# CPJKU/audio_sheet_retrieval

Measured on AMD Instinct MI355X. Metric: snippet-pairs/sec embedded+ranked (32-d CCA), higher is better.
Workload: dtype f32

## Files before the change

### audio_sheet_retrieval_amd/csrc/asr_api.hip

```cpp
#include "asr_ctx.h"


namespace asr_detail {

thread_local std::string g_create_error;

int fail(asr_ctx *ctx, int code, const char *fmt, ...) {
    char buf[512];
    va_list ap;
    va_start(ap, fmt);
    vsnprintf(buf, sizeof buf, fmt, ap);
    va_end(ap);
    if (ctx) ctx->err = buf; else g_create_error = buf;
    return code;
}


void build_geometry(Tower &t, int nf, int H, int W) {
    const int ch[9][2] = {{1, nf}, {nf, nf}, {nf, 2 * nf}, {2 * nf, 2 * nf}, {2 * nf, 4 * nf},
                          {4 * nf, 4 * nf}, {4 * nf, 4 * nf}, {4 * nf, 4 * nf}, {4 * nf, 32}};
    t.in_h = H; t.in_w = W;
    int h = H, w = W;
    for (int b = 0; b < 9; ++b) {
        LayerGeom &g = t.g[b];
// ... 98 lines not shown
    if (T.mask) hipFree(T.mask);
    if (T.raw1) hipFree(T.raw1);
    if (T.repack_dev) hipFree(T.repack_dev);
    if (T.cca_ws) hipFree(T.cca_ws);
    if (T.l2_dev) hipFree(T.l2_dev);
    if (T.cca_done) hipEventDestroy(T.cca_done);
    for (hipEvent_t e : T.gate) if (e) hipEventDestroy(e);
    ctx->train.reset();
}

void free_comm(asr_ctx *ctx) {
    if (!ctx->comm) return;
    Comm &c = *ctx->comm;
    for (auto &pr : c.timed) { (void)hipEventDestroy(pr.first); (void)hipEventDestroy(pr.second); }
    c.timed.clear();
    if (c.nccl && c.pCommDestroy) (void)c.pCommDestroy(c.nccl);
    if (c.dl) dlclose(c.dl);
    ctx->comm.reset();
    ctx->exch = asr::Exchange{};
}

void free_pipe(asr_ctx *ctx) {
    auto &P = ctx->pipe;
    for (int s = 0; s < 2; ++s) {
        void *bufs[] = {P.in1[s], P.in2[s], P.lv1[s], P.lv2[s], P.ranks[s], P.ties[s], P.dstar[s]};
        for (void *b : bufs) if (b) (void)hipFree(b);
        hipEvent_t evs[] = {P.ready[s], P.done[s], P.out[s]};
        for (hipEvent_t e : evs) if (e) (void)hipEventDestroy(e);
    }
    if (P.h2d && P.h2d != ctx->copy_streams[0]) (void)hipStreamDestroy(P.h2d);
    if (P.d2h && P.d2h != ctx->copy_streams[1]) (void)hipStreamDestroy(P.d2h);
    P = asr_ctx::Pipe{};
}

void free_hpipe(asr_ctx *ctx) {
    auto &H = ctx->hpipe;
    for (int s = 0; s < asr_ctx::HostPipe::NSLOT; ++s) {
        if (H.pin[s]) (void)hipHostFree(H.pin[s]);
        if (H.dev[s]) (void)hipFree(H.dev[s]);
        if (H.copied[s]) (void)hipEventDestroy(H.copied[s]);
        if (H.consumed[s]) (void)hipEventDestroy(H.consumed[s]);
        H.pin[s] = H.dev[s] = nullptr; H.copied[s] = H.consumed[s] = nullptr; H.used[s] = false;
    }
    H.slot_bytes = 0;
    if (H.out_dev) (void)hipFree(H.out_dev);
    H.out_dev = nullptr; H.out_floats = 0;
    if (H.h2d && H.h2d != ctx->copy_streams[2]) (void)hipStreamDestroy(H.h2d);
    H.h2d = nullptr;
    H.pool.reset();
}

void free_ctx_buffers(asr_ctx *ctx) {
    free_train(ctx);
    free_comm(ctx);
    free_pipe(ctx);
    free_hpipe(ctx);
    for (auto &t : ctx->tw) {
        for (int b = 0; b < 9; ++b) { if (t.w_dev[b]) hipFree(t.w_dev[b]); if (t.bn_dev[b]) hipFree(t.bn_dev[b]); }
        for (int b = 0; b < 8; ++b) if (t.act[b]) hipFree(t.act[b]);
    }
    if (ctx->cca_dev) hipFree(ctx->cca_dev);
    for (int v = 0; v < 2; ++v) {
        if (ctx->in_stage[v]) hipFree(ctx->in_stage[v]);
        if (ctx->out_stage[v]) hipFree(ctx->out_stage[v]);
        if (ctx->vdone[v]) hipEventDestroy(ctx->vdone[v]);
        if (ctx->vstream[v]) hipStreamDestroy(ctx->vstream[v]);
    }
    if (ctx->main_done) hipEventDestroy(ctx->main_done);
    if (ctx->wside_stream) { (void)hipStreamSynchronize(ctx->wside_stream); (void)hipStreamDestroy(ctx->wside_stream); }
    for (hipStream_t &cs : ctx->copy_streams)
        if (cs) { (void)hipStreamSynchronize(cs); (void)hipStreamDestroy(cs); cs = nullptr; }
    if (ctx->norm1) hipFree(ctx->norm1);
    if (ctx->norm2) hipFree(ctx->norm2);
    if (ctx->cca_ws) hipFree(ctx->cca_ws);
    if (ctx->topk_ws) hipFree(ctx->topk_ws);
    if (ctx->topk_tickets) hipFree(ctx->topk_tickets);
    if (ctx->unit_ws) hipFree(ctx->unit_ws);
    if (ctx->rank_io) hipFree(ctx->rank_io);
    if (ctx->valid_ws) hipFree(ctx->valid_ws);
    for (auto &r : ctx->prof) prof_fold(r.get());
    if (ctx->stream) hipStreamDestroy(ctx->stream);
}

hipError_t launch_conv_any(asr_ctx *ctx, hipStream_t st, const asr::ConvPlan &p, const float *in, const float *w,
                           const float *bn, float *out, int n, const asr::Fuse1Args *f1, double *stats, int *stats_rows,
                           bool stats_clean, const asr::BnBwdFuse *bf) {
    if (stats_rows) *stats_rows = 0;
    if (p.variant >= 4000)
        return asr::launch_conv_wino4(st, p, in, w + asr::conv_wpack_floats(p.cin, p.cout) + asr::wino_wpack_floats(p.cin, p.cout),
                                      bn, out, n, ctx->num_cus, stats, stats_rows, stats_clean, bf);
    if (p.variant >= 3000)
        return asr::launch_conv_wino(st, p, in, w + asr::conv_wpack_floats(p.cin, p.cout), bn, out, n, ctx->num_cus,
                                     stats, stats_rows, p.fuse1 ? f1 : nullptr, stats_clean, bf);
    if (p.variant >= 2000) return asr::launch_conv_v3(st, p, in, w, bn, out, n, ctx->num_cus, p.fuse1 ? f1 : nullptr);
    return p.variant >= 1000 ? asr::launch_conv_v2(st, p, in, w, bn, out, n, ctx->num_cus)
                             : asr::launch_conv(st, p, in, w, bn, out, n, ctx->num_cus, f1);
}

int tune_cache_tag() {
    static int tag = -1;
    if (tag < 0) {
        unsigned h = 2166136261u;
        for (const char *p = asr_version(); *p; ++p) h = (h ^ (unsigned char)*p) * 16777619u;
        tag = (int)(h & 0x7fffffffu);
    }
    return tag;
}

int autotune_tower(asr_ctx *ctx, int view) {
    Tower &t = ctx->tw[view - 1];
    hipStream_t st = ctx->estream[view - 1];
    const int n = ctx->chunk;
    hipEvent_t e0, e1;
    ASR_HIP(ctx, hipEventCreate(&e0));
    ASR_HIP(ctx, hipEventCreate(&e1));
    const bool dbg = getenv("ASR_DEBUG") != nullptr;
    for (int b = 1; b < 8; ++b) {
        const LayerGeom &g = t.g[b];
        std::vector<asr::ConvPlan> cands;
        cands.push_back(t.plan[b]);
        const char *fenv = getenv("ASR_FUSE1");
        const bool forced = (b == 1 && t.fuse1);
        const bool try_fused = (b == 1) && fenv && fenv[0] != '0' && fenv[0] != 'w' && getenv("ASR_NO_FUSE1") == nullptr;
        const bool try_wfused = (b == 1) && !(fenv && fenv[0] == '0') && getenv("ASR_NO_FUSE1") == nullptr &&
                                !(view == 1 && ctx->cfg.resize_view1) && !forced;
        const bool only_wfused = try_wfused && fenv && fenv[0] == 'w';
        if (!forced) {
            asr::conv_candidates_v1(g.cin, g.cout, g.pool, g.H, g.W, 0, 5, &cands, 0);
            asr::conv_candidates_v2(g.cin, g.cout, g.pool, g.H, g.W, 5, &cands);
            asr::conv_candidates_v3(g.cin, g.cout, g.pool, g.H, g.W, 6, &cands, 0);
            asr::conv_candidates_wino(g.cin, g.cout, g.pool, g.H, g.W,
                                      getenv("ASR_WINO_CANDS") ? atoi(getenv("ASR_WINO_CANDS")) : 4, &cands);
            asr::conv_candidates_wino4(g.cin, g.cout, g.pool, g.H, g.W, &cands);
        } else {
            asr::conv_candidates_v1(g.cin, g.cout, g.pool, g.H, g.W, 0, 5, &cands, 1);
        }
        if (try_fused) asr::conv_candidates_v3(g.cin, g.cout, g.pool, g.H, g.W, 6, &cands, 1);
        if (try_wfused) {
            asr::conv_candidates_wino_fused(g.cin, g.cout, g.pool, g.H, g.W, 3, &cands);
            if (only_wfused) {
                std::vector<asr::ConvPlan> only;
                for (auto &c : cands)
                    if (c.variant >= 3000 && c.variant < 3500 && c.fuse1) only.push_back(c);
                if (!only.empty()) cands.swap(only);
            }
        }
        if (b == 1 && fenv && fenv[0] == '3') {
            std::vector<asr::ConvPlan> only;
            for (auto &c : cands)
                if (c.variant >= 2000 && c.fuse1) only.push_back(c);
            if (!only.empty()) cands.swap(only);
        }
        if (const char *only_env = getenv("ASR_TUNE_ONLY")) {
            const int lo = !strcmp(only_env, "wino4") ? 4000 : !strcmp(only_env, "winog") ? 3500 : !strcmp(only_env, "wino") ? 3000 : 0;
            const int hi = !strcmp(only_env, "wino4") ? 5000 : !strcmp(only_env, "winog") ? 4000 : !strcmp(only_env, "wino") ? 3500 : 3000;
            std::vector<asr::ConvPlan> only;
            for (auto &c : cands)
                if (c.variant >= lo && c.variant < hi) only.push_back(c);
            if (!only.empty()) cands.swap(only);
        }
        asr::Fuse1Args f1{t.act[0], t.w_dev[0], t.bn_dev[0], ASR_IN_F32_PREPARED, 0, g.H, g.W};
        const asr::Fuse1Args *pf1 = &f1;
        double conv1_ms = 0.0;
        bool any_fused = false;
        for (auto &c : cands) any_fused = any_fused || c.fuse1;
        if (b == 1 && any_fused && !forced) {
            const LayerGeom &g0 = t.g[0];
            ASR_HIP(ctx, hipMemsetD32Async((hipDeviceptr_t)t.act[1], 0x3f000000, (size_t)g0.H * g0.W * n, st));
            (void)asr::launch_conv1(st, t.act[1], ASR_IN_F32_PREPARED, 0, t.w_dev[0], t.bn_dev[0], t.act[0], n, g0.H, g0.W,
                                    g0.H, g0.W, g0.cout);
            ASR_HIP(ctx, hipEventRecord(e0, st));
            for (int r = 0; r < 2; ++r)
                (void)asr::launch_conv1(st, t.act[1], ASR_IN_F32_PREPARED, 0, t.w_dev[0], t.bn_dev[0], t.act[0], n, g0.H,
                                        g0.W, g0.H, g0.W, g0.cout);
            ASR_HIP(ctx, hipEventRecord(e1, st));
            ASR_HIP(ctx, hipEventSynchronize(e1));
            float ms = 0.f;
            ASR_HIP(ctx, hipEventElapsedTime(&ms, e0, e1));
            conv1_ms = ms / 2;
            if (dbg) fprintf(stderr, "[asr] tune v%d conv1 alone: %.4f ms\n", view, conv1_ms);
        }
        const bool verify = getenv("ASR_TUNE_VERIFY") != nullptr;
        const size_t out_floats = t.act_floats[b] * (size_t)n;
        float *vref = nullptr;
        uint32_t *vbits = nullptr;
        bool have_ref = false;
        if (verify) {
            ASR_HIP(ctx, asr::launch_fill_pattern(st, t.act[b - 1], (int64_t)t.act_floats[b - 1] * n));
            ASR_HIP(ctx, hipMalloc((void **)&vref, out_floats * sizeof(float) + 16));
            vbits = reinterpret_cast<uint32_t *>(vref + out_floats);
        } else
        ASR_HIP(ctx, hipMemsetD32Async((hipDeviceptr_t)t.act[b - 1], 0x3f000000, t.act_floats[b - 1] * n, st));
        double best_ms = 1e30;
        int best = -1;
        const char *cache = getenv("ASR_TUNE_CACHE");
        const int nf = ctx->cfg.num_filters;
        if (cache) {
            if (FILE *fp = fopen(cache, "r")) {
                char line[256];
                while (fgets(line, sizeof line, fp)) {
                    int k[10], tag = 0;
                    if (sscanf(line, "v2 %d %d %d %d %d %d %d %d %d %d %d", &tag, &k[0], &k[1], &k[2], &k[3], &k[4], &k[5],
                               &k[6], &k[7], &k[8], &k[9]) != 11 || tag != tune_cache_tag())
                        continue;
                    if (k[0] != nf || k[1] != view || k[2] != b || k[3] != g.H || k[4] != g.W || k[5] != n) continue;
                    for (size_t c = 0; c < cands.size(); ++c)
                        if (cands[c].variant == k[6] && cands[c].TH == k[7] && cands[c].TW == k[8] && cands[c].NI == k[9])
                            best = (int)c;
                }
                fclose(fp);
            }
        }
        if (best >= 0) {
            t.plan[b] = cands[best];
            if (b == 1) t.fuse1 = cands[best].fuse1 != 0;
            if (dbg) fprintf(stderr, "[asr] tuned v%d conv%d from cache%s\n", view, b + 1, t.fuse1 && b == 1 ? " (fused)" : "");
            continue;
        }
        best = 0;
        for (size_t c = 0; c < cands.size(); ++c) {
            hipError_t e = launch_conv_any(ctx, st, cands[c], t.act[b - 1], t.w_dev[b], t.bn_dev[b], t.act[b], n, pf1);
            if (e != hipSuccess) { (void)hipGetLastError(); continue; }
            if (verify && !cands[c].fuse1) {
                if (!have_ref) {
                    ASR_HIP(ctx, hipMemcpyAsync(vref, t.act[b], out_floats * sizeof(float), hipMemcpyDeviceToDevice, st));
                    have_ref = true;
                } else {
                    uint32_t bits = 0;
                    ASR_HIP(ctx, asr::launch_max_abs_diff(st, t.act[b], vref, (int64_t)out_floats, vbits));
                    ASR_HIP(ctx, hipMemcpyAsync(&bits, vbits, sizeof bits, hipMemcpyDeviceToHost, st));
                    ASR_HIP(ctx, hipStreamSynchronize(st));
                    float diff;
                    memcpy(&diff, &bits, sizeof diff);
                    ctx->tune_checked += 1;
                    if (!(diff <= (cands[c].variant >= 3000 ? 1e-4f : 1e-5f))) {
                        ctx->tune_bad += 1;
                        fprintf(stderr, "[asr] TUNE VERIFY MISMATCH view %d conv%d variant %d tile %dx%d x%d: max |diff| %g\n",
                                view, b + 1, cands[c].variant, cands[c].TH, cands[c].TW, cands[c].NI, (double)diff);
                    }
                    if (diff > ctx->tune_max_diff || diff != diff) ctx->tune_max_diff = diff;
                }
                ASR_HIP(ctx, hipMemsetAsync(t.act[b], 0xff, out_floats * sizeof(float), st));
                (void)launch_conv_any(ctx, st, cands[c], t.act[b - 1], t.w_dev[b], t.bn_dev[b], t.act[b], n, pf1);
            }
            ASR_HIP(ctx, hipEventRecord(e0, st));
            for (int r = 0; r < 2; ++r)
                (void)launch_conv_any(ctx, st, cands[c], t.act[b - 1], t.w_dev[b], t.bn_dev[b], t.act[b], n, pf1);
            ASR_HIP(ctx, hipEventRecord(e1, st));
            ASR_HIP(ctx, hipEventSynchronize(e1));
            float ms = 0.f;
            ASR_HIP(ctx, hipEventElapsedTime(&ms, e0, e1));
            if (dbg)
                fprintf(stderr, "[asr] tune v%d conv%d%s %s#%d tile %dx%d x%d lds %d bpc %d: %.4f ms\n", view, b + 1,
                        cands[c].fuse1 ? "+1" : "",
                        cands[c].variant >= 4000 ? "wino4" : cands[c].variant >= 3000 ? "wino" : cands[c].variant >= 2000 ? "v3" : cands[c].variant >= 1000 ? "v2" : "v1",
                        cands[c].variant % 1000, cands[c].TH, cands[c].TW,
                        cands[c].NI, cands[c].lds_bytes, cands[c].blocks_per_cu, ms / 2);
            const bool rowmajor_winog = cands[c].variant >= 3500 && cands[c].variant < 4000 && cands[c].TH == 1;
            const double cost = (ms / 2) * (rowmajor_winog ? 1.02 : 1.0) + (cands[c].fuse1 ? 0.0 : conv1_ms);
            if (cost < best_ms) { best_ms = cost; best = (int)c; }
        }
        if (vref) (void)hipFree(vref);
        t.plan[b] = cands[best];
        if (b == 1) t.fuse1 = cands[best].fuse1 != 0;
        if (cache) {
            if (FILE *fp = fopen(cache, "a")) {
                fprintf(fp, "v2 %d %d %d %d %d %d %d %d %d %d %d\n", tune_cache_tag(), nf, view, b, g.H, g.W, n,
                        cands[best].variant, cands[best].TH, cands[best].TW, cands[best].NI);
                fclose(fp);
            }
        }
        if (dbg)
            fprintf(stderr, "[asr] tuned v%d conv%d -> %s#%d tile %dx%d x%d (%.4f ms for %d samples)\n", view, b + 1,
                    cands[best].variant >= 4000 ? "wino4" : cands[best].variant >= 3000 ? "wino" : cands[best].variant >= 2000 ? "v3" : cands[best].variant >= 1000 ? "v2" : "v1",
                    cands[best].variant % 1000, cands[best].TH,
                    cands[best].TW, cands[best].NI, best_ms, n);
    }
    (void)hipEventDestroy(e0);
    (void)hipEventDestroy(e1);
    return ASR_OK;
}

int ensure_workspace(asr_ctx *ctx, int view) {
    Tower &t = ctx->tw[view - 1];
    for (int b = 0; b < 8; ++b)
        if (!t.act[b]) ASR_HIP(ctx, hipMalloc((void **)&t.act[b], t.act_floats[b] * ctx->chunk * sizeof(float)));
    if (!t.tuned) {
        t.tuned = true;
        const char *e = getenv("ASR_AUTOTUNE");
        if (!(e && e[0] == '0')) return autotune_tower(ctx, view);
    }
    return ASR_OK;
}

int ensure_staging(asr_ctx *ctx, int view) {
    const int v = view - 1;
    if (!ctx->in_stage[v]) ASR_HIP(ctx, hipMalloc(&ctx->in_stage[v], ctx->in_stage_bytes));
    if (!ctx->out_stage[v])
        ASR_HIP(ctx, hipMalloc((void **)&ctx->out_stage[v], (size_t)ctx->chunk * 32 * sizeof(float)));
    return ASR_OK;
}

int join_views(asr_ctx *ctx) {
    for (int v = 0; v < 2; ++v)
        if (ctx->vpending[v]) {
            ASR_HIP(ctx, hipStreamWaitEvent(ctx->stream, ctx->vdone[v], 0));
            ctx->vpending[v] = false;
        }
    return ASR_OK;
}

int mark_main(asr_ctx *ctx) {
    ASR_HIP(ctx, hipEventRecord(ctx->main_done, ctx->stream));
    ctx->main_pending = true;
    return ASR_OK;
}

int sync_all(asr_ctx *ctx) {
    for (int v = 0; v < 2; ++v) ASR_HIP(ctx, hipStreamSynchronize(ctx->vstream[v]));
    ASR_HIP(ctx, hipStreamSynchronize(ctx->stream));
    ctx->vpending[0] = ctx->vpending[1] = false;
    ctx->main_pending = false;
    return ASR_OK;
}


int run_tower(asr_ctx *ctx, int view, const void *x_dev, int in_mode, int n, float *features_dev, float *latent_dev) {
    Tower &t = ctx->tw[view - 1];
    const asr_config &c = ctx->cfg;
    hipStream_t st = ctx->estream[view - 1];
    const int rsz = (view == 1) ? c.resize_view1 : 0;
    const int hraw = (view == 1) ? c.h1 : c.h2, wraw = (view == 1) ? c.w1 : c.w2;
    if (!t.fuse1) {
        const LayerGeom &g = t.g[0];
        ProfScope ps(ctx, "conv1", view, 2.0 * n * g.H * g.W * 9.0 * g.cout,
                     (double)n * g.H * g.W * (4.0 + 4.0 * g.cout), asr::conv1_symbol(g.cout, in_mode, rsz, n, g.H, g.W, hraw, wraw));
        ASR_HIP(ctx, asr::launch_conv1(st, x_dev, in_mode, rsz, t.w_dev[0], t.bn_dev[0], t.act[0], n, hraw,
                                       wraw, g.H, g.W, g.cout));
    }
    for (int b = 1; b < 8; ++b) {
        const LayerGeom &g = t.g[b];
        const bool fused = (b == 1 && t.fuse1);
        char name[32];
        snprintf(name, sizeof name, fused ? "conv1+%d" : "conv%d", b + 1);
        ProfScope ps(ctx, name, view,
                     2.0 * n * g.H * g.W * 9.0 * g.cin * g.cout + (fused ? 2.0 * n * g.H * g.W * 9.0 * g.cin : 0.0),
                     4.0 * n * ((double)g.H * g.W * (fused ? 1 : g.cin) + (double)g.OH * g.OW * g.cout),
                     fused ? asr::conv_wino_symbol(t.plan[b], in_mode) : t.plan[b].symbol);
        asr::Fuse1Args f1{x_dev, t.w_dev[0], t.bn_dev[0], in_mode, rsz, hraw, wraw};
        ASR_HIP(ctx, launch_conv_any(ctx, st, t.plan[b], t.act[b - 1], t.w_dev[b], t.bn_dev[b], t.act[b], n,
                                     fused ? &f1 : nullptr));
    }
    {
        const LayerGeom &g = t.g[8];
        ProfScope ps(ctx, "tail", view, 2.0 * n * (g.H * g.W * (double)g.cin * 32 + 32.0 * 32),
                     4.0 * n * ((double)g.H * g.W * g.cin + 64));
        const float *mean = ctx->cca_dev + 2048 + (view == 1 ? 0 : 32);
        const float *proj = ctx->cca_dev + (view == 1 ? 0 : 1024);
        ASR_HIP(ctx, asr::launch_tail(st, t.act[7], n, g.H, g.W, g.cin, t.w_dev[8], t.bn_dev[8], mean, proj,
                                      features_dev, latent_dev));
    }
    ctx->last_n[view - 1] = n;
    return ASR_OK;
}

size_t input_bytes_per_sample(const asr_ctx *ctx, int view, int in_mode) {
    const asr_config &c = ctx->cfg;
    if (view == 2) return (size_t)c.h2 * c.w2 * 4;
    if (in_mode == ASR_IN_F32_PREPARED) return (size_t)ctx->tw[0].in_h * ctx->tw[0].in_w * 4;
    return (size_t)c.h1 * c.w1 * (in_mode == ASR_IN_U8_RAW ? 1 : 4);
}

int embed_common(asr_ctx *ctx, int view, const void *x, int in_mode, int64_t n, int out_kind, float *out,
                 bool on_device) {
    if (!ctx) return ASR_ERR_INVALID;
    if (!ctx->params_set) return fail(ctx, ASR_ERR_STATE, "embed: asr_set_params has not been called");
    if (n < 0 || (n > 0 && (!x || !out))) return fail(ctx, ASR_ERR_INVALID, "embed: NULL buffer or negative n");
    if (in_mode < 0 || in_mode > 2 || (view == 2 && in_mode != ASR_IN_F32_PREPARED))
        return fail(ctx, ASR_ERR_INVALID, "embed: bad in_mode %d for view %d", in_mode, view);
    if (out_kind != ASR_OUT_LATENT && out_kind != ASR_OUT_FEATURES)
        return fail(ctx, ASR_ERR_INVALID, "embed: bad out_kind %d", out_kind);
    ASR_HIP(ctx, hipSetDevice(ctx->cfg.device));
    if (n > 0) {
        int rcw = ensure_workspace(ctx, view);
        if (rcw != ASR_OK) return rcw;
    }
    if (ctx->wino_stale) {
        int rcr = refresh_wino_weights(ctx);
        if (rcr != ASR_OK) return rcr;
    }
    const size_t bps = input_bytes_per_sample(ctx, view, in_mode);
    hipStream_t st = ctx->estream[view - 1];
    if (n > 0 && !on_device) {
        int rcs = ensure_staging(ctx, view);
        if (rcs != ASR_OK) return rcs;
    }
    if (n > 0 && on_device && ctx->main_pending)
        ASR_HIP(ctx, hipStreamWaitEvent(st, ctx->main_done, 0));
    for (int64_t s0 = 0; s0 < n; s0 += ctx->chunk) {
        const int nc = (int)std::min<int64_t>(ctx->chunk, n - s0);
        const void *xin;
        float *o;
        if (on_device) {
            xin = (const char *)x + (size_t)s0 * bps;
            o = out + (size_t)s0 * 32;
        } else {
            ASR_HIP(ctx, hipMemcpyAsync(ctx->in_stage[view - 1], (const char *)x + (size_t)s0 * bps,
                                        (size_t)nc * bps, hipMemcpyHostToDevice, st));
            xin = ctx->in_stage[view - 1];
            o = ctx->out_stage[view - 1];
        }
        int rc = run_tower(ctx, view, xin, in_mode, nc, out_kind == ASR_OUT_FEATURES ? o : nullptr,
                           out_kind == ASR_OUT_LATENT ? o : nullptr);
        if (rc != ASR_OK) return rc;
        if (!on_device) {
            ASR_HIP(ctx, hipMemcpyAsync(out + (size_t)s0 * 32, o, (size_t)nc * 32 * sizeof(float),
                                        hipMemcpyDeviceToHost, st));
            ASR_HIP(ctx, hipStreamSynchronize(st));
        }
    }
    if (n > 0 && on_device) {
        ASR_HIP(ctx, hipEventRecord(ctx->vdone[view - 1], st));
        ctx->vpending[view - 1] = true;
    }
    return ASR_OK;
}

// ... 797 lines not shown
```

### audio_sheet_retrieval_amd/csrc/conv_wino4_kernels.hip

```cpp
#include <hip/hip_runtime.h>
#include <stdint.h>
#include <stdlib.h>
#include <algorithm>
#include <type_traits>
#include <vector>
#include "asr_kernels.h"
#include "repack_elems.inl"

#ifndef ASR_WINO4_ABL
#define ASR_WINO4_ABL 0
#endif

namespace asr {

typedef float floatx4q __attribute__((ext_vector_type(4)));
typedef float float2q __attribute__((ext_vector_type(2)));

struct Wino4Args {
    const float *in, *wpk, *bnp;
    float *out;
    int N, H, W, OH, OW;
    int ty_img, tx_img;
    int coutp;
    int tiles;
// ... 373 lines not shown
            }
        }
        unsigned voff[9];
#pragma unroll
        for (int k = 0; k < 9; ++k) {
            voff[k] = wlane + (unsigned)k * (2 * wstep * 16);
            asm volatile("" : "+v"(voff[k]));
        }
        floatx4q acc[36];
        auto reload = [&](const float *wn, auto set_c) {
            constexpr int SET = decltype(set_c)::value;
            if (ASR_WINO4_ABL & 4) return;
            const char *wnb = reinterpret_cast<const char *>(wn);
#pragma unroll
            for (int k = 0; k < 9; ++k) {
                unsigned vo = voff[k];
                asm volatile("" : "+v"(vo));
                bw[SET][2 * k] = *reinterpret_cast<const floatx4q *>(wnb + vo);
                bw[SET][2 * k + 1] = *reinterpret_cast<const floatx4q *>(wnb + (wstep * 16) + vo);
            }
        };
        auto run_step = [&](const float *vb, const float *wn, auto cur_c, auto first) {
            constexpr bool FIRST = decltype(first)::value;
            constexpr int CUR = decltype(cur_c)::value;
            using NXT = std::integral_constant<int, CUR ^ 1>;
            __syncthreads();
            reload(wn, NXT{});
            __builtin_amdgcn_sched_barrier(0);
            float2q dp[2][12];
#pragma unroll
            for (int i = 0; i < 12; ++i) dp[0][i] = *reinterpret_cast<const float2q *>(vb + i * 128);
#pragma unroll
            for (int grp = 0; grp < 3; ++grp) {
                if (grp < 2) {
#pragma unroll
                    for (int i = 0; i < 12; ++i)
                        dp[(grp + 1) & 1][i] = *reinterpret_cast<const float2q *>(vb + ((grp + 1) * 12 + i) * 128);
                }
#pragma unroll
                for (int c = 0; c < 2; ++c)
#pragma unroll
                    for (int i = 0; i < 12; ++i) {
                        const int p = grp * 12 + i;
                        if (FIRST && c == 0)
                            acc[p] = __builtin_amdgcn_mfma_f32_16x16x4f32(dp[grp & 1][i][c], bw[CUR][(c * 36 + p) >> 2][(c * 36 + p) & 3],
                                                                          floatx4q{0.f, 0.f, 0.f, 0.f}, 0, 0, 0);
                        else
                            acc[p] = __builtin_amdgcn_mfma_f32_16x16x4f32(dp[grp & 1][i][c], bw[CUR][(c * 36 + p) >> 2][(c * 36 + p) & 3], acc[p],
                                                                          0, 0,
                                                                          0);
                    }
                __builtin_amdgcn_sched_barrier(0);
            }
        };
        using C0 = std::integral_constant<int, 0>;
        using C1 = std::integral_constant<int, 1>;
        auto wblock = [&](int t) {
            unsigned blk = (unsigned)(((t + 1) % NB) * 72) * wstep;
            asm volatile("" : "+s"(blk));
            return wl + blk;
        };
        run_step(vlane + (step & 1) * VB, wblock(0), C0{}, std::true_type{});
        ++step;
#pragma unroll 1
        for (int t = 1; t + 1 < NB; t += 2) {
            run_step(vlane + (step & 1) * VB, wblock(t), C1{}, std::false_type{});
            ++step;
            run_step(vlane + (step & 1) * VB, wblock(t + 1), C0{}, std::false_type{});
            ++step;
        }
        if constexpr ((NB & 1) == 0) {
            run_step(vlane + (step & 1) * VB, wblock(NB - 1), C1{}, std::false_type{});
            ++step;
        } else {
#pragma unroll
            for (int j = 0; j < 18; ++j) bw[0][j] = bw[1][j];
        }

        unsigned eo[4];
        int ee[4];
#pragma unroll
        for (int r = 0; r < 4; ++r) {
            eo[r] = (unsigned)__shfl((int)my_off, 4 * g + r);
            ee[r] = __shfl(my_ext, 4 * g + r);
        }
        if (!ch_ok) continue;
        floatx4q tc[4][6];
#pragma unroll
        for (int nu = 0; nu < 6; ++nu)
            out6(acc[nu], acc[6 + nu], acc[12 + nu], acc[18 + nu], acc[24 + nu], acc[30 + nu], tc[0][nu], tc[1][nu], tc[2][nu],
                 tc[3][nu]);
        if (POOL) {
#pragma unroll
            for (int pr = 0; pr < 2; ++pr) {
                floatx4q ya[4], yb[4];
                out6(tc[2 * pr][0], tc[2 * pr][1], tc[2 * pr][2], tc[2 * pr][3], tc[2 * pr][4], tc[2 * pr][5], ya[0], ya[1],
                     ya[2], ya[3]);
                out6(tc[2 * pr + 1][0], tc[2 * pr + 1][1], tc[2 * pr + 1][2], tc[2 * pr + 1][3], tc[2 * pr + 1][4],
                     tc[2 * pr + 1][5], yb[0], yb[1], yb[2], yb[3]);
#pragma unroll
                for (int pc = 0; pc < 2; ++pc) {
#pragma unroll
                    for (int r = 0; r < 4; ++r) {
                        if (pr >= (ee[r] & 0xff) || pc >= (ee[r] >> 8)) continue;
                        const float v0 = ya[2 * pc][r], v1 = ya[2 * pc + 1][r], v2 = yb[2 * pc][r], v3 = yb[2 * pc + 1][r];
                        const float hi = fmaxf(fmaxf(v0, v1), fmaxf(v2, v3));
                        const float lo = fminf(fminf(v0, v1), fminf(v2, v3));
                        const float x = bscale >= 0.0f ? hi : lo;
                        const float res = elu_fastq((x - bmean) * bscale + bbeta);
                        if (ASR_WINO4_ABL & 32) asm volatile("" ::"v"(res));
                        else a.out[(size_t)eo[r] + (size_t)(pr * a.OW + pc) * COUT + chn] = res;
                    }
                }
            }
        } else {
#pragma unroll
            for (int i = 0; i < 4; ++i) {
                floatx4q y[4];
                out6(tc[i][0], tc[i][1], tc[i][2], tc[i][3], tc[i][4], tc[i][5], y[0], y[1], y[2], y[3]);
                float rs1 = 0.f, rs2 = 0.f;
#pragma unroll
                for (int j = 0; j < 4; ++j) {
#pragma unroll
                    for (int r = 0; r < 4; ++r) {
                        if (i >= (ee[r] & 0xff) || j >= (ee[r] >> 8)) continue;
                        const float res = RAW ? y[j][r] : elu_fastq((y[j][r] - bmean) * bscale + bbeta);
                        if (RAW) {
                            if (bnb) {
                                const size_t e = (size_t)eo[r] + (size_t)(i * a.W + j) * COUT + chn;
                                bnb_acc(res, a.bf.z[e], bnb_mult(a.bf.tie, e), bmean, bscale, bbeta, bistd, rs1, rs2);
                            } else { rs1 += res; rs2 = fmaf(res, res, rs2); }
                        }
                        if (ASR_WINO4_ABL & 32) asm volatile("" ::"v"(res));
                        else a.out[(size_t)eo[r] + (size_t)(i * a.W + j) * COUT + chn] = res;
                    }
                }
                if (RAW) { st1 += (double)rs1; st2 += (double)rs2; }
            }
        }
    }
    __syncthreads();
    if constexpr (RAW) {
        if (a.stats) {
            st1 += __shfl_xor(st1, 16); st2 += __shfl_xor(st2, 16);
            st1 += __shfl_xor(st1, 32); st2 += __shfl_xor(st2, 32);
            if (g == 0 && ch_ok) {
                a.stats[((size_t)blockIdx.x * 2) * COUT + chn] = st1;
                a.stats[((size_t)blockIdx.x * 2 + 1) * COUT + chn] = st2;
            }
        }
    }
}

__global__ void wino4_pack_kernel(const float *W, int cin, int cout, int dgrad, float *wpk) {
    const int idx = blockIdx.x * blockDim.x + threadIdx.x;
    if (idx >= wino4_pack_count(cin, cout, dgrad)) return;
    wino4_pack_elem(idx, W, cin, cout, dgrad, wpk);
}

size_t wino4_wpack_floats(int cin, int cout) { return (cin % 8) ? 0 : (size_t)36 * cin * ((cout + 15) / 16 * 16); }

hipError_t launch_wino4_pack(hipStream_t s, const float *W, int cin, int cout, float *wpk, int dgrad) {
    const int kdim = dgrad ? cout : cin, ndim = dgrad ? cin : cout;
    if (kdim % 8) return hipSuccess;
    const int total = kdim * ((ndim + 15) / 16 * 16);
    hipLaunchKernelGGL(wino4_pack_kernel, dim3((total + 255) / 256), dim3(256), 0, s, W, cin, cout, dgrad, wpk);
    return hipGetLastError();
}

struct Wino4Variant {
    int cin, cout, pool, waves, raw;
    void (*kernel)(Wino4Args);
    const char *symbol;
    int spec;
    int slice;
};
#define ASR_BOOLSTRQ_0 "false"
#define ASR_BOOLSTRQ_1 "true"
#define ASR_WINO4(CIN, COUT, POOL, WAVES)                                                                         \
    { CIN, COUT, POOL, WAVES, 0, conv3x3_wino4g<CIN, COUT, (POOL != 0), WAVES, false>,                            \
      "void asr::conv3x3_wino4g<" #CIN ", " #COUT ", " ASR_BOOLSTRQ_##POOL ", " #WAVES ", false>(asr::Wino4Args)" }
#define ASR_WINO4S(CIN, COUT, POOL)                                                                               \
    { CIN, COUT, POOL, 1 + (COUT + 15) / 16, 0, conv3x3_wino4s<CIN, COUT, (POOL != 0)>,                           \
      "void asr::conv3x3_wino4s<" #CIN ", " #COUT ", " ASR_BOOLSTRQ_##POOL ", " #COUT ", 1, false>(asr::Wino4Args)", 1, 0 }
#define ASR_WINO4S2(CIN, COUT, POOL)                                                                              \
    { CIN, COUT, POOL, 2 + (COUT + 15) / 16, 0, conv3x3_wino4s<CIN, COUT, (POOL != 0), COUT, 2>,                  \
      "void asr::conv3x3_wino4s<" #CIN ", " #COUT ", " ASR_BOOLSTRQ_##POOL ", " #COUT ", 2, false>(asr::Wino4Args)", 1, 0 }
#define ASR_WINO4SR(CIN, COUT)                                                                                    \
    { CIN, COUT, 0, 1 + (COUT + 15) / 16, 1, conv3x3_wino4s<CIN, COUT, false, COUT, 1, true>,                     \
      "void asr::conv3x3_wino4s<" #CIN ", " #COUT ", false, " #COUT ", 1, true>(asr::Wino4Args)", 1, 0 }
#define ASR_WINO4SL(CIN, COUT, POOL, SLICE)                                                                       \
    { CIN, COUT, POOL, 1 + SLICE / 16, 0, conv3x3_wino4s<CIN, COUT, (POOL != 0), SLICE>,                          \
      "void asr::conv3x3_wino4s<" #CIN ", " #COUT ", " ASR_BOOLSTRQ_##POOL ", " #SLICE ", 1, false>(asr::Wino4Args)", 1, SLICE }
static const Wino4Variant g_wino4[] = {
    ASR_WINO4(24, 24, 1, 4), ASR_WINO4(24, 48, 0, 4), ASR_WINO4(48, 48, 1, 4), ASR_WINO4(48, 48, 0, 4),
    ASR_WINO4S(24, 24, 1), ASR_WINO4S(24, 48, 0), ASR_WINO4S(48, 48, 1), ASR_WINO4S(48, 48, 0),
    ASR_WINO4S2(24, 24, 1),
    ASR_WINO4SL(48, 96, 0, 48), ASR_WINO4SL(96, 96, 1, 48), ASR_WINO4SL(96, 96, 0, 48),
    ASR_WINO4SR(24, 48), ASR_WINO4SR(48, 48), ASR_WINO4SR(48, 24),
};
static const int g_num_wino4 = (int)(sizeof(g_wino4) / sizeof(g_wino4[0]));

void conv_candidates_wino4(int cin, int cout, int pool, int H, int W, std::vector<ConvPlan> *out) {
    static const int use = getenv("ASR_CONV_WINO4") ? atoi(getenv("ASR_CONV_WINO4")) : -1;
    if (use == 0) return;
    for (int vi = 0; vi < g_num_wino4; ++vi) {
        const Wino4Variant &v = g_wino4[vi];
        if (v.cin != cin || v.cout != cout || v.pool != pool || v.raw) continue;
        if (!v.spec && use != 1) continue;
        const int lds = v.spec ? 2 * 36 * 16 * 8 * 4 : 36 * cin * 16 * 4;
        (void)hipFuncSetAttribute(reinterpret_cast<const void *>(v.kernel), hipFuncAttributeMaxDynamicSharedMemorySize,
                                  160 * 1024);
        int nb = 0;
        if (hipOccupancyMaxActiveBlocksPerMultiprocessor(&nb, reinterpret_cast<const void *>(v.kernel), 64 * v.waves,
                                                         (size_t)lds) != hipSuccess || nb < 1) {
            (void)hipGetLastError();
            nb = 1;
        }
        ConvPlan bp{};
        bp.cin = cin; bp.cout = cout; bp.pool = pool;
        bp.H = H; bp.W = W; bp.OH = pool ? H / 2 : H; bp.OW = pool ? W / 2 : W;
        bp.TH = 4; bp.TW = 64; bp.NI = 16;
        bp.tiles_y = (H + 3) / 4; bp.tiles_x = (W + 3) / 4;
        bp.threads = 64 * v.waves;
        bp.lds_bytes = lds;
        bp.blocks_per_cu = v.spec ? 1 : std::min(nb, 4);
        bp.cost = (double)bp.tiles_y * bp.tiles_x / 16.0 * ((cout + 15) / 16) * (36.0 * (cin / 4) * 32.0 + 3000.0) *
                  (v.spec ? 0.4 : 1.0);
        bp.variant = 4000 + vi;
        bp.symbol = v.symbol;
        out->push_back(bp);
    }
}

void conv_candidates_wino4_raw(int cin, int cout, int H, int W, std::vector<ConvPlan> *out, int dgrad) {
    static const int use = getenv("ASR_TRAIN_WINO4") ? atoi(getenv("ASR_TRAIN_WINO4")) : -1;
    if (use == 0 || (use == 5 && !dgrad)) return;
    for (int vi = 0; vi < g_num_wino4; ++vi) {
        const Wino4Variant &v = g_wino4[vi];
        if (v.cin != cin || v.cout != cout || !v.raw) continue;
        const int lds = 2 * 36 * 16 * 8 * 4;
        (void)hipFuncSetAttribute(reinterpret_cast<const void *>(v.kernel), hipFuncAttributeMaxDynamicSharedMemorySize,
                                  160 * 1024);
        ConvPlan bp{};
        bp.cin = cin; bp.cout = cout; bp.pool = 0;
        bp.H = H; bp.W = W; bp.OH = H; bp.OW = W;
        bp.TH = 4; bp.TW = 64; bp.NI = 16;
        bp.tiles_y = (H + 3) / 4; bp.tiles_x = (W + 3) / 4;
        bp.threads = 64 * v.waves;
        bp.lds_bytes = lds;
        bp.blocks_per_cu = 1;
        bp.cost = (double)bp.tiles_y * bp.tiles_x / 16.0 * ((cout + 15) / 16) * (36.0 * (cin / 4) * 32.0 + 3000.0) * 0.4;
        bp.variant = 4000 + vi;
        bp.symbol = v.symbol;
        out->push_back(bp);
    }
}
bool conv_wino4_is_raw(const ConvPlan &p) { return p.variant >= 4000 && g_wino4[p.variant - 4000].raw != 0; }
int conv_wino4_stats_rows_max(int num_cus) { return num_cus; }

hipError_t launch_conv_wino4(hipStream_t s, const ConvPlan &p, const float *in, const float *wpk, const float *bnp,
                             float *out, int N, int num_cus, double *stats, int *stats_rows, bool stats_clean,
                             const BnBwdFuse *bf) {
    const Wino4Variant &v = g_wino4[p.variant - 4000];
    Wino4Args a;
    a.stats = nullptr;
    a.bf = BnBwdFuse{nullptr, nullptr, nullptr};
    a.in = in; a.wpk = wpk; a.bnp = bnp; a.out = out;
    a.N = N; a.H = p.H; a.W = p.W; a.OH = p.OH; a.OW = p.OW;
    a.ty_img = p.tiles_y; a.tx_img = p.tiles_x;
    a.coutp = (p.cout + 15) / 16 * 16;
    a.tiles = N * a.ty_img * a.tx_img;
    a.total = (a.tiles + 15) / 16;
    if (a.total == 0) return hipSuccess;
    if (v.spec) {
        if ((double)N * p.H * p.W * p.cin * 4.0 >= 4294967296.0) return hipErrorInvalidValue;
        const int slices = v.slice ? p.cout / v.slice : 1;
        int grid = std::min(a.total, std::max(1, num_cus * std::max(1, p.blocks_per_cu) / slices));
        if (grid >= 8) grid &= ~7;
        if (v.raw && stats) {
            a.stats = stats;
            if (bf) a.bf = *bf;
            (void)stats_clean;
            if (stats_rows) *stats_rows = grid;
        }
        hipLaunchKernelGGL(v.kernel, dim3(grid, slices), dim3(p.threads), p.lds_bytes, s, a);
        return hipGetLastError();
    }
    const int ntiles = a.coutp / 16;
    const int waves = p.threads / 64;
    const int slots = std::max(1, num_cus * std::max(1, p.blocks_per_cu) / ntiles);
    const int grid = std::min((a.total + waves - 1) / waves, slots);
    hipLaunchKernelGGL(v.kernel, dim3(grid, ntiles), dim3(p.threads), p.lds_bytes, s, a);
    return hipGetLastError();
}

}
```

Before: 290,200.

## Add large-tile Winograd F(4,3) conv kernel for 12-channel layers with LDS DMA prefetch

Adds a new Winograd 4x4 conv kernel for 12-input-channel layers. Each block processes multi-16x16 macro-tiles, stages inputs into double-buffered LDS via buffer_load...lds DMA and prefetches the next region, and computes with MFMA 16x16x4 fp32, with BN+ELU and optional max-pool fused into the epilogue. The kernel is registered as autotuner candidates (variant 5000+), so it is used only when the tuner measures it as faster. Weight packing is relaxed to allow cin divisible by 4. This adds considerable kernel complexity and relies on padded LDS row strides that are checked for bank conflicts.

```diff
diff --git a/audio_sheet_retrieval_amd/csrc/asr_api.hip b/audio_sheet_retrieval_amd/csrc/asr_api.hip
--- a/audio_sheet_retrieval_amd/csrc/asr_api.hip
+++ b/audio_sheet_retrieval_amd/csrc/asr_api.hip
@@ -274,8 +274,8 @@
             if (!only.empty()) cands.swap(only);
         }
         if (const char *only_env = getenv("ASR_TUNE_ONLY")) {
-            const int lo = !strcmp(only_env, "wino4") ? 4000 : !strcmp(only_env, "winog") ? 3500 : !strcmp(only_env, "wino") ? 3000 : 0;
-            const int hi = !strcmp(only_env, "wino4") ? 5000 : !strcmp(only_env, "winog") ? 4000 : !strcmp(only_env, "wino") ? 3500 : 3000;
+            const int lo = !strcmp(only_env, "wino4l") ? 5000 : !strcmp(only_env, "wino4") ? 4000 : !strcmp(only_env, "winog") ? 3500 : !strcmp(only_env, "wino") ? 3000 : 0;
+            const int hi = !strcmp(only_env, "wino4l") ? 6000 : !strcmp(only_env, "wino4") ? 5000 : !strcmp(only_env, "winog") ? 4000 : !strcmp(only_env, "wino") ? 3500 : 3000;
             std::vector<asr::ConvPlan> only;
             for (auto &c : cands)
                 if (c.variant >= lo && c.variant < hi) only.push_back(c);
@@ -375,7 +375,7 @@
             if (dbg)
                 fprintf(stderr, "[asr] tune v%d conv%d%s %s#%d tile %dx%d x%d lds %d bpc %d: %.4f ms\n", view, b + 1,
                         cands[c].fuse1 ? "+1" : "",
-                        cands[c].variant >= 4000 ? "wino4" : cands[c].variant >= 3000 ? "wino" : cands[c].variant >= 2000 ? "v3" : cands[c].variant >= 1000 ? "v2" : "v1",
+                        cands[c].variant >= 5000 ? "wino4l" : cands[c].variant >= 4000 ? "wino4" : cands[c].variant >= 3000 ? "wino" : cands[c].variant >= 2000 ? "v3" : cands[c].variant >= 1000 ? "v2" : "v1",
                         cands[c].variant % 1000, cands[c].TH, cands[c].TW,
                         cands[c].NI, cands[c].lds_bytes, cands[c].blocks_per_cu, ms / 2);
             const bool rowmajor_winog = cands[c].variant >= 3500 && cands[c].variant < 4000 && cands[c].TH == 1;
@@ -394,7 +394,7 @@
         }
         if (dbg)
             fprintf(stderr, "[asr] tuned v%d conv%d -> %s#%d tile %dx%d x%d (%.4f ms for %d samples)\n", view, b + 1,
-                    cands[best].variant >= 4000 ? "wino4" : cands[best].variant >= 3000 ? "wino" : cands[best].variant >= 2000 ? "v3" : cands[best].variant >= 1000 ? "v2" : "v1",
+                    cands[best].variant >= 5000 ? "wino4l" : cands[best].variant >= 4000 ? "wino4" : cands[best].variant >= 3000 ? "wino" : cands[best].variant >= 2000 ? "v3" : cands[best].variant >= 1000 ? "v2" : "v1",
                     cands[best].variant % 1000, cands[best].TH,
                     cands[best].TW, cands[best].NI, best_ms, n);
     }
diff --git a/audio_sheet_retrieval_amd/csrc/conv_wino4_kernels.hip b/audio_sheet_retrieval_amd/csrc/conv_wino4_kernels.hip
--- a/audio_sheet_retrieval_amd/csrc/conv_wino4_kernels.hip
+++ b/audio_sheet_retrieval_amd/csrc/conv_wino4_kernels.hip
@@ -549,17 +549,322 @@
     }
 }
 
+struct Wino4LArgs {
+    const float *in, *wpk, *bnp;
+    float *out;
+    int N, H, W, OH, OW;
+    int nmy, nmx;
+    int tiles_y, tiles_x;
+    int coutp;
+    int RP;
+    int total, per;
+};
+
+template <> __device__ __forceinline__ float splatq<float>(float c) { return c; }
+template <typename T> __device__ __forceinline__ void out6_lo(T m0, T m1, T m2, T m3, T m4, T &y0, T &y1) {
+    const T s1 = m1 + m2, s2 = m1 - m2, s3 = m3 + m4, s4 = m3 - m4;
+    y0 = (m0 + s1) + s3;
+    y1 = fmaq(2.f, s4, s2);
+}
+template <typename T> __device__ __forceinline__ void out6_hi(T m1, T m2, T m3, T m4, T m5, T &y2, T &y3) {
+    const T s1 = m1 + m2, s2 = m1 - m2, s3 = m3 + m4, s4 = m3 - m4;
+    y2 = fmaq(4.f, s3, s1);
+    y3 = fmaq(8.f, s4, s2) + m5;
+}
+typedef __attribute__((address_space(3))) float lds_float;
+__device__ float g_wino4l_sink[64];
+
+constexpr int wino4l_w_floats(int cout) {
+    return (27 * 4 * ((cout + 15) / 16 == 1 ? 16 : cout) * 4 + 255) & ~255;
+}
+
+template <int CIN, int COUT, bool POOL, int WAVES, int RMAX>
+__global__ __launch_bounds__(64 * WAVES, 1) void conv3x3_wino4l(Wino4LArgs a) {
+    static_assert(CIN == 12, "one 8-channel block and a 4-channel remainder");
+    constexpr int NT = (COUT + 15) / 16;
+    constexpr int WSC = NT == 1 ? 16 : COUT;
+    constexpr int NQ = 27;
+    constexpr int CSf = 12;
+    constexpr int T = 64 * WAVES;
+    constexpr int WD = 2;
+    constexpr int WF = wino4l_w_floats(COUT);
+    extern __shared__ __align__(16) float lds[];
+    const int tid = threadIdx.x, lane = tid & 63;
+    const int wave = __builtin_amdgcn_readfirstlane(tid >> 6);
+    const int nmt = a.nmy * a.nmx;
+    const int LW = a.nmx * 16 + 2, LH = a.nmy * 16 + 2;
+    const int RPf = a.RP * 4;
+    const int buf_floats = (LH * RPf + 255) & ~255;
+    lds_float *const pbuf = (lds_float *)lds + WF;
+    const int first = blockIdx.x * a.per;
+    const int last = min(first + a.per, a.total);
+    if (first >= last) return;
+
+    for (int i = tid; i < NQ * 4 * WSC; i += T) {
+        const int rg = i / WSC, col = i - rg * WSC;
+        *reinterpret_cast<floatx4q *>(lds + i * 4) =
+            *reinterpret_cast<const floatx4q *>(a.wpk + ((size_t)rg * a.coutp + col) * 4);
+    }
+    constexpr int RH = (RMAX + 1) / 2;
+    unsigned st[RH];
+#pragma unroll
+    for (int k = 0; k < RH; ++k) st[k] = 0;
+#pragma unroll
+    for (int k = 0; k < RMAX; ++k) {
+        const int f = tid + k * T;
+        const int r = f / a.RP;
+        const int xs = f - r * a.RP - ((r >> 2) & 3);
+        const bool real = r < LH && xs >= 0 && xs < 3 * LW;
+        st[k >> 1] |= (real ? (unsigned)(r << 9 | xs) : 511u) << (16 * (k & 1));
+    }
+    typedef int int4v __attribute__((ext_vector_type(4)));
+    auto fetch = [&](int region, lds_float *buf) __attribute__((always_inline)) {
+        const int tx = region % a.tiles_x;
+        const int rest = region / a.tiles_x;
+        const int ty = rest % a.tiles_y;
+        const int img = rest / a.tiles_y;
+        const int Y0 = ty * a.nmy * 16, X0 = tx * a.nmx * 16;
+        const uint64_t ibase = reinterpret_cast<uint64_t>(a.in + (int64_t)img * a.H * a.W * CIN);
+        int4v rsrc;
+        rsrc.x = (int)(uint32_t)ibase;
+        rsrc.y = (int)(uint32_t)(ibase >> 32);
+        rsrc.z = a.H * a.W * CIN * 4;
+        rsrc.w = 0x00020000;
+        const int roff = (Y0 * a.W + X0 - a.W - 1) * CIN * 4;
+        const unsigned lds0 = (unsigned)(uintptr_t)buf;
+        auto dma = [&](int k, int vo) __attribute__((always_inline)) {
+            const unsigned m0v = lds0 + (unsigned)((k * T + wave * 64) * 16);
+            asm volatile("s_mov_b32 m0, %2\n\ts_nop 0\n\tbuffer_load_dwordx4 %0, %1, 0 offen lds"
+                         ::"v"(vo), "s"(rsrc), "s"(m0v)
+                         : "memory", "m0");
+        };
+        const int xlo = max(0, 3 - 3 * X0), xhi = min(3 * LW, 3 * (a.W - X0 + 1));
+        const int rowb = 3 * a.W * 16;
+#pragma unroll
+        for (int k = 0; k < RMAX; ++k) {
+            if ((k * T + wave * 64) * 4 >= buf_floats) break;
+            const unsigned e = (st[k >> 1] >> (16 * (k & 1))) & 0xffffu;
+            const int r = (int)(e >> 9), xs = (int)(e & 511u);
+            const int off = r * rowb + xs * 16 + roff;
+            dma(k, (xs >= xlo && xs < xhi) ? off : (int)0x80000000);
+        }
+    };
+    fetch(first, pbuf);
+    asm volatile("s_waitcnt vmcnt(0)" ::: "memory");
+    __syncthreads();
+    if (first + 1 < last) fetch(first + 1, pbuf + buf_floats);
+
+    const int m = lane & 15, g = lane >> 4, n = lane & 15;
+    const int tyy = m >> 2, txx = m & 3;
+    int a_row[6];
+#pragma unroll
+    for (int i = 0; i < 6; ++i) a_row[i] = (4 * tyy + i) * RPf + ((tyy + (i >> 2)) & 3) * 4 + 4 * txx * CSf + 2 * g;
+    const int a_rem = 8 - g;
+    const lds_float *const w_lane = (const lds_float *)lds + (g * WSC + n) * 4;
+    float bmean[NT], bscale[NT], bbeta[NT];
+#pragma unroll
+    for (int nt = 0; nt < NT; ++nt) {
+        const int ch = nt * 16 + n;
+        const bool ok = ch < COUT;
+        bmean[nt] = ok ? a.bnp[ch] : 0.f;
+        bscale[nt] = ok ? a.bnp[a.coutp + ch] : 1.f;
+        bbeta[nt] = ok ? a.bnp[2 * a.coutp + ch] : 0.f;
+    }
+
+    auto region_origin = [&](int region, int &img, int &Y0, int &X0) __attribute__((always_inline)) {
+        const int tx = region % a.tiles_x;
+        const int rest = region / a.tiles_x;
+        const int ty = rest % a.tiles_y;
+        img = rest / a.tiles_y;
+        Y0 = ty * a.nmy * 16; X0 = tx * a.nmx * 16;
+    };
+    auto find = [&](int region, int from) __attribute__((always_inline)) {
+        int img, Y0, X0;
+        region_origin(region, img, Y0, X0);
+        for (int mt = from; mt < nmt; mt += WAVES) {
+            const int mty = mt / a.nmx, mtx = mt - mty * a.nmx;
+            if (Y0 + 16 * mty < a.H && X0 + 16 * mtx < a.W) return mt;
+        }
+        return -1;
+    };
+    int pending_fetch = -1;
+    auto issue_pending = [&]() __attribute__((always_inline)) {
+        if (pending_fetch >= 0) fetch(pending_fetch, pbuf + ((pending_fetch - first) & 1) * buf_floats);
+        pending_fetch = -1;
+    };
+    auto transition = [&](int region) __attribute__((always_inline)) {
+        issue_pending();
+        asm volatile("s_waitcnt vmcnt(0)" ::: "memory");
+        __syncthreads();
+        if (region + 2 < last) pending_fetch = region + 2;
+    };
+    auto mtile_base = [&](int region, int mt) __attribute__((always_inline)) -> const lds_float * {
+        const int mty = mt / a.nmx, mtx = mt - mty * a.nmx;
+        return pbuf + ((region - first) & 1) * buf_floats + 16 * mty * RPf + 16 * mtx * CSf;
+    };
+
+    float2q pq[6][6];
+    const lds_float *cur = nullptr;
+    auto pread = [&](int idx, const lds_float *base) __attribute__((always_inline)) {
+        const int i = idx / 6, j = idx % 6;
+        pq[i][j] = *(const volatile __attribute__((address_space(3))) float2q *)(base + a_row[i] + j * CSf);
+    };
+
+    int reg = first, mt = find(first, wave);
+    while (mt < 0) {
+        if (reg + 1 >= last) { reg = last; break; }
+        transition(reg);
+        issue_pending();
+        ++reg;
+        mt = find(reg, wave);
+    }
+    if (reg < last) {
+        cur = mtile_base(reg, mt);
+#pragma unroll
+        for (int idx = 0; idx < 36; ++idx) pread(idx, cur);
+    }
+    floatx4q bpre[WD];
+#pragma unroll
+    for (int q = 0; q < WD; ++q) bpre[q] = *(const __attribute__((address_space(3))) floatx4q *)(w_lane + q * 4 * WSC * 4);
+
+    while (reg < last) {
+        float2q dp[6][6];
+        float dr[6][6];
+#pragma unroll
+        for (int i = 0; i < 6; ++i)
+#pragma unroll
+            for (int j = 0; j < 6; ++j) dr[i][j] = *(const volatile lds_float *)(cur + a_row[i] + a_rem + j * CSf);
+#pragma unroll
+        for (int i = 0; i < 6; ++i)
+#pragma unroll
+            for (int j = 0; j < 6; ++j) dp[i][j] = pq[i][j];
+#pragma unroll
+        for (int j = 0; j < 6; ++j) in6(dp[0][j], dp[1][j], dp[2][j], dp[3][j], dp[4][j], dp[5][j]);
+#pragma unroll
+        for (int i = 0; i < 6; ++i) in6(dp[i][0], dp[i][1], dp[i][2], dp[i][3], dp[i][4], dp[i][5]);
+#pragma unroll
+        for (int j = 0; j < 6; ++j) in6(dr[0][j], dr[1][j], dr[2][j], dr[3][j], dr[4][j], dr[5][j]);
+#pragma unroll
+        for (int i = 0; i < 6; ++i) in6(dr[i][0], dr[i][1], dr[i][2], dr[i][3], dr[i][4], dr[i][5]);
+        int img, Y0, X0;
+        region_origin(reg, img, Y0, X0);
+        const int mty = mt / a.nmx, mtx = mt - mty * a.nmx;
+        const int py0 = Y0 + 16 * mty, px0 = X0 + 16 * mtx;
+        int nreg = reg, nmt_ = find(reg, mt + WAVES);
+        while (nmt_ < 0) {
+            if (nreg + 1 >= last) { nreg = last; break; }
+            transition(nreg);
+            ++nreg;
+            nmt_ = find(nreg, wave);
+        }
+        const lds_float *nb = nreg < last ? mtile_base(nreg, nmt_) : mtile_base(reg, mt);
+
+        floatx4q bw[NQ + WD];
+#pragma unroll
+        for (int q = 0; q < WD; ++q) bw[q] = bpre[q];
+#pragma unroll
+        for (int nt = 0; nt < NT; ++nt) {
+            floatx4q acc[36];
+            typedef const __attribute__((address_space(3))) floatx4q lds_f4;
+            const lds_float *wk = w_lane + nt * 16 * 4;
+            const lds_float *wn = nt + 1 < NT ? wk + 16 * 4 : w_lane;
+#pragma unroll
+            for (int R = 0; R < NQ; ++R) {
+                bw[R + WD] = (R + WD < NQ) ? *(lds_f4 *)(wk + (R + WD) * 4 * WSC * 4)
+                                           : *(lds_f4 *)(wn + (R + WD - NQ) * 4 * WSC * 4);
+                if (nt == NT - 1 && R < 18) {
+#pragma unroll
+                    for (int idx = 2 * R; idx < 2 * R + 2; ++idx) pread(idx, nb);
+                }
+                __builtin_amdgcn_sched_barrier(0);
+#pragma unroll
+                for (int e = 0; e < 4; ++e) {
+                    const int row = 4 * R + e;
+                    float av;
+                    int p;
+                    if (row < 72) { p = row % 36; av = dp[p / 6][p % 6][row / 36]; }
+                    else { p = row - 72; av = dr[p / 6][p % 6]; }
+                    if (row < 36)
+                        acc[p] = __builtin_amdgcn_mfma_f32_16x16x4f32(av, bw[R][e], floatx4q{0.f, 0.f, 0.f, 0.f}, 0, 0, 0);
+                    else
+                        acc[p] = __builtin_amdgcn_mfma_f32_16x16x4f32(av, bw[R][e], acc[p], 0, 0, 0);
+                }
+                __builtin_amdgcn_sched_barrier(0);
+            }
+#pragma unroll
+            for (int q = 0; q < WD; ++q) bw[q] = bw[NQ + q];
+
+            const int ch = nt * 16 + n;
+            if (ch >= COUT) continue;
+            floatx4q tc[4][6];
+#pragma unroll
+            for (int nu = 0; nu < 6; ++nu)
+                out6(acc[nu], acc[6 + nu], acc[12 + nu], acc[18 + nu], acc[24 + nu], acc[30 + nu], tc[0][nu], tc[1][nu],
+                     tc[2][nu], tc[3][nu]);
+            if (POOL) {
+                const int qy0 = py0 >> 1, qx0 = px0 >> 1;
+                float *ob = a.out + (((int64_t)img * a.OH + qy0) * a.OW + qx0) * COUT + ch;
+                const int ly = a.OH - qy0, lx = a.OW - qx0;
+#pragma unroll
+                for (int pr = 0; pr < 2; ++pr) {
+                    floatx4q ya[4], yb[4];
+                    out6(tc[2 * pr][0], tc[2 * pr][1], tc[2 * pr][2], tc[2 * pr][3], tc[2 * pr][4], tc[2 * pr][5], ya[0],
+                         ya[1], ya[2], ya[3]);
+                    out6(tc[2 * pr + 1][0], tc[2 * pr + 1][1], tc[2 * pr + 1][2], tc[2 * pr + 1][3], tc[2 * pr + 1][4],
+                         tc[2 * pr + 1][5], yb[0], yb[1], yb[2], yb[3]);
+                    const int oy = 2 * g + pr;
+#pragma unroll
+                    for (int r = 0; r < 4; ++r)
+#pragma unroll
+                        for (int pc = 0; pc < 2; ++pc) {
+                            const int ox = 2 * r + pc;
+                            const float v0 = ya[2 * pc][r], v1 = ya[2 * pc + 1][r], v2 = yb[2 * pc][r], v3 = yb[2 * pc + 1][r];
+                            const float hi = fmaxf(fmaxf(v0, v1), fmaxf(v2, v3));
+                            const float lo = fminf(fminf(v0, v1), fminf(v2, v3));
+                            const float x = bscale[nt] >= 0.0f ? hi : lo;
+                            float *dst = (oy < ly && ox < lx) ? ob + (oy * a.OW + ox) * COUT : g_wino4l_sink + lane;
+                            *dst = elu_fastq((x - bmean[nt]) * bscale[nt] + bbeta[nt]);
+                        }
+                }
+            } else {
+                float *ob = a.out + (((int64_t)img * a.H + py0) * a.W + px0) * COUT + ch;
+                const int ly = a.H - py0, lx = a.W - px0;
+#pragma unroll
+                for (int i = 0; i < 4; ++i) {
+                    floatx4q y[4];
+                    out6(tc[i][0], tc[i][1], tc[i][2], tc[i][3], tc[i][4], tc[i][5], y[0], y[1], y[2], y[3]);
+                    const int oy = 4 * g + i;
+#pragma unroll
+                    for (int r = 0; r < 4; ++r)
+#pragma unroll
+                        for (int j = 0; j < 4; ++j) {
+                            const int ox = 4 * r + j;
+                            float *dst = (oy < ly && ox < lx) ? ob + (oy * a.W + ox) * COUT : g_wino4l_sink + lane;
+                            *dst = elu_fastq((y[j][r] - bmean[nt]) * bscale[nt] + bbeta[nt]);
+                        }
+                }
+            }
+        }
+#pragma unroll
+        for (int q = 0; q < WD; ++q) bpre[q] = bw[q];
+        issue_pending();
+        reg = nreg;
+        mt = nmt_;
+        cur = nb;
+    }
+}
+
 __global__ void wino4_pack_kernel(const float *W, int cin, int cout, int dgrad, float *wpk) {
     const int idx = blockIdx.x * blockDim.x + threadIdx.x;
     if (idx >= wino4_pack_count(cin, cout, dgrad)) return;
     wino4_pack_elem(idx, W, cin, cout, dgrad, wpk);
 }
 
-size_t wino4_wpack_floats(int cin, int cout) { return (cin % 8) ? 0 : (size_t)36 * cin * ((cout + 15) / 16 * 16); }
+size_t wino4_wpack_floats(int cin, int cout) { return (cin % 4) ? 0 : (size_t)36 * cin * ((cout + 15) / 16 * 16); }
 
 hipError_t launch_wino4_pack(hipStream_t s, const float *W, int cin, int cout, float *wpk, int dgrad) {
     const int kdim = dgrad ? cout : cin, ndim = dgrad ? cin : cout;
-    if (kdim % 8) return hipSuccess;
+    if (kdim % 8 && (dgrad || kdim % 4)) return hipSuccess;
     const int total = kdim * ((ndim + 15) / 16 * 16);
     hipLaunchKernelGGL(wino4_pack_kernel, dim3((total + 255) / 256), dim3(256), 0, s, W, cin, cout, dgrad, wpk);
     return hipGetLastError();
@@ -598,9 +903,104 @@
 };
 static const int g_num_wino4 = (int)(sizeof(g_wino4) / sizeof(g_wino4[0]));
 
+struct Wino4LVariant {
+    int cin, cout, pool, rmax;
+    void (*kernel)(Wino4LArgs);
+    const char *symbol;
+};
+#define ASR_WINO4L(CIN, COUT, POOL, RMAX)                                                                         \
+    { CIN, COUT, POOL, RMAX, conv3x3_wino4l<CIN, COUT, (POOL != 0), 4, RMAX>,                                     \
+      "void asr::conv3x3_wino4l<" #CIN ", " #COUT ", " ASR_BOOLSTRQ_##POOL ", 4, " #RMAX ">(asr::Wino4LArgs)" }
+static const Wino4LVariant g_wino4l[] = {
+    ASR_WINO4L(12, 12, 1, 15), ASR_WINO4L(12, 24, 0, 15),
+};
+static const int g_num_wino4l = (int)(sizeof(g_wino4l) / sizeof(g_wino4l[0]));
+
+int wino4l_lds_conflicts(int rp) {
+    int worst = 1;
+    for (int i = 0; i < 6; ++i)
+        for (int j = 0; j < 6; ++j)
+            for (int kind = 0; kind < 2; ++kind)
+                for (int half = 0; half < 2; ++half) {
+                    int seen[64][64], nseen[64] = {0};
+                    for (int l = 0; l < 32; ++l) {
+                        const int lane = half * 32 + l, m = lane & 15, g = lane >> 4, tyy = m >> 2, txx = m & 3;
+                        const int row = ((4 * tyy + i) * rp + ((tyy + (i >> 2)) & 3)) * 4 + (4 * txx + j) * 12;
+                        const int d0 = row + (kind == 0 ? 2 * g : 8 + g);
+                        for (int w = 0; w < (kind == 0 ? 2 : 1); ++w) {
+                            const int d = d0 + w, bank = d & 63;
+                            bool dup = false;
+                            for (int q = 0; q < nseen[bank]; ++q) dup = dup || seen[bank][q] == d;
+                            if (!dup) seen[bank][nseen[bank]++] = d;
+                            worst = std::max(worst, nseen[bank]);
+                        }
+                    }
+                }
+    return worst;
+}
+
+static void candidates_wino4l(int cin, int cout, int pool, int H, int W, std::vector<ConvPlan> *out) {
+    static const int use = getenv("ASR_CONV_WINO4L") ? atoi(getenv("ASR_CONV_WINO4L")) : 1;
+    if (!use) return;
+    static const int shapes[3][2] = {{1, 4}, {2, 2}, {4, 1}};
+    for (int vi = 0; vi < g_num_wino4l; ++vi) {
+        const Wino4LVariant &v = g_wino4l[vi];
+        if (v.cin != cin || v.cout != cout || v.pool != pool) continue;
+        if ((double)(H + 2) * W * 3 >= 4194304.0 || (double)H * W * cin * 4.0 >= 134217728.0) continue;
+        (void)hipFuncSetAttribute(reinterpret_cast<const void *>(v.kernel), hipFuncAttributeMaxDynamicSharedMemorySize,
+                                  160 * 1024);
+        for (const auto &sh : shapes) {
+            const int nmy = sh[0], nmx = sh[1];
+            const int LH = 16 * nmy + 2, LW = 16 * nmx + 2;
+            const int rp = 3 * LW + 3;
+            const int buf_bytes = ((LH * rp * 16) + 1023) & ~1023;
+            const int lds = wino4l_w_floats(cout) * 4 + 2 * buf_bytes;
+            if (lds > 160 * 1024 || LH * rp > v.rmax * 256) continue;
+            if (wino4l_lds_conflicts(rp) != 1) continue;
+            const int tiles_y = (H + 16 * nmy - 1) / (16 * nmy), tiles_x = (W + 16 * nmx - 1) / (16 * nmx);
+            ConvPlan bp{};
+            bp.cin = cin; bp.cout = cout; bp.pool = pool;
+            bp.H = H; bp.W = W; bp.OH = pool ? H / 2 : H; bp.OW = pool ? W / 2 : W;
+            bp.TH = 16 * nmy; bp.TW = 16 * nmx; bp.NI = nmy;
+            bp.tiles_y = tiles_y; bp.tiles_x = tiles_x;
+            bp.threads = 256;
+            bp.lds_bytes = lds;
+            bp.blocks_per_cu = 1;
+            bp.tile_floats = nmy * 1000 + nmx;
+            bp.rp = rp; bp.c4p = 3;
+            bp.cost = (double)tiles_y * tiles_x * (108.0 * ((cout + 15) / 16) * 32.0 + 1800.0 + 1200.0);
+            bp.variant = 5000 + vi;
+            bp.symbol = v.symbol;
+            out->push_back(bp);
+        }
+    }
+}
+
+static hipError_t launch_conv_wino4l(hipStream_t s, const ConvPlan &p, const float *in, const float *wpk,
+                                     const float *bnp, float *out, int N, int num_cus) {
+    const Wino4LVariant &v = g_wino4l[p.variant - 5000];
+    if ((double)(p.TH + 2) * p.W * 3 >= 4194304.0 || (double)p.H * p.W * p.cin * 4.0 >= 134217728.0)
+        return hipErrorInvalidValue;
+    Wino4LArgs a;
+    a.in = in; a.wpk = wpk; a.bnp = bnp; a.out = out;
+    a.N = N; a.H = p.H; a.W = p.W; a.OH = p.OH; a.OW = p.OW;
+    a.nmy = p.tile_floats / 1000; a.nmx = p.tile_floats % 1000;
+    a.tiles_y = p.tiles_y; a.tiles_x = p.tiles_x;
+    a.coutp = (p.cout + 15) / 16 * 16;
+    a.RP = p.rp;
+    a.total = N * p.tiles_y * p.tiles_x;
+    if (a.total == 0) return hipSuccess;
+    const int slots = std::max(1, num_cus * std::max(1, p.blocks_per_cu));
+    a.per = (a.total + slots - 1) / slots;
+    const int grid = (a.total + a.per - 1) / a.per;
+    hipLaunchKernelGGL(v.kernel, dim3(grid), dim3(p.threads), p.lds_bytes, s, a);
+    return hipGetLastError();
+}
+
 void conv_candidates_wino4(int cin, int cout, int pool, int H, int W, std::vector<ConvPlan> *out) {
     static const int use = getenv("ASR_CONV_WINO4") ? atoi(getenv("ASR_CONV_WINO4")) : -1;
     if (use == 0) return;
+    candidates_wino4l(cin, cout, pool, H, W, out);
     for (int vi = 0; vi < g_num_wino4; ++vi) {
         const Wino4Variant &v = g_wino4[vi];
         if (v.cin != cin || v.cout != cout || v.pool != pool || v.raw) continue;
@@ -653,12 +1053,15 @@
         out->push_back(bp);
     }
 }
-bool conv_wino4_is_raw(const ConvPlan &p) { return p.variant >= 4000 && g_wino4[p.variant - 4000].raw != 0; }
+bool conv_wino4_is_raw(const ConvPlan &p) {
+    return p.variant >= 4000 && p.variant < 5000 && g_wino4[p.variant - 4000].raw != 0;
+}
 int conv_wino4_stats_rows_max(int num_cus) { return num_cus; }
 
 hipError_t launch_conv_wino4(hipStream_t s, const ConvPlan &p, const float *in, const float *wpk, const float *bnp,
                              float *out, int N, int num_cus, double *stats, int *stats_rows, bool stats_clean,
                              const BnBwdFuse *bf) {
+    if (p.variant >= 5000) return launch_conv_wino4l(s, p, in, wpk, bnp, out, N, num_cus);
     const Wino4Variant &v = g_wino4[p.variant - 4000];
     Wino4Args a;
     a.stats = nullptr;
```

Result: no change. 290,000 (median of 4 runs) (-0.1%).
